# yeyupiaoling/MASR

Hardware: AMD Instinct MI355X
Metric: audio-seconds/sec (RTF^-1), conformer_streaming_fbank b32x10s, PCM->fbank->encoder->ctc_greedy->text (higher is better)
Workload: dtype f32; 1 GPU; configs[1]: conformer.yml streaming fbank, batch=32 synthetic 16 kHz 10 s utterances per GPU, ctc_greedy, random-init weights V=4233; global_batch=32, parallelism=dp1, world_size_observed=1, backend=none

## Files before the change

include/masr_hip.h:

```cpp
#ifndef MASR_HIP_H
#define MASR_HIP_H
#include <stdint.h>
#ifdef __cplusplus
extern "C" {
#endif

typedef struct masr_engine masr_engine;

typedef struct masr_config {
    int32_t model_kind;
    int32_t d_model;
    int32_t heads;
    int32_t d_ff;
    int32_t num_blocks;
    int32_t cnn_kernel;
    int32_t n_mels;
    int32_t vocab_size;
    int32_t causal;
    int32_t max_pos;
    int32_t device_id;
    int32_t reserved[5];
} masr_config;

const char* masr_last_error(void);
// ... 174 lines not shown
int masr_resample_plan(const masr_resample_feed* feeds, int32_t n_feeds, const masr_resample_rate* rates, int32_t n_rates,
                       int64_t src_bytes, int32_t dst_rows, int64_t dst_stride, int32_t* tiles, int64_t tiles_cap, int64_t* n_tiles,
                       int32_t* bad_feed, const char** why);
int masr_resample_feeds(masr_engine* e, const void* src_dev, int64_t src_bytes, const masr_resample_feed* feeds_host,
                        const masr_resample_feed* feeds_dev, int32_t n_feeds, const masr_resample_rate* rates_host,
                        const masr_resample_rate* rates_dev, int32_t n_rates, const int32_t* tiles_host, const int32_t* tiles_dev,
                        int64_t n_tiles, float* dst_dev, int32_t dst_rows, int64_t dst_stride, void* stream);
int masr_encode_chunk(masr_engine* e, const int32_t* stream_ids, int32_t n, const float* feats_dev, int32_t Tc,
                      float* probs_dev, int32_t* argmax_dev, float* maxprob_dev, void* stream);
int masr_stream_export_cache(masr_engine* e, int32_t stream_id, float* att_dev, float* cnn_dev, void* stream);

int masr_op_layernorm(masr_engine* e, const float* x_dev, const float* w_dev, const float* b_dev, float* y_dev,
                      int32_t M, float eps, void* stream);
int masr_op_gemm(masr_engine* e, const float* a_dev, const float* w_dev, const float* bias_dev, const float* res_dev,
                 float* c_dev, int32_t M, int32_t N, int32_t K, int32_t act, float alpha, void* stream);
int masr_op_ctc_collapse_rows(masr_engine* e, const int32_t* argmax_dev, const float* maxprob_dev, const int32_t* n_frames_dev,
                              const int32_t* in_rows_dev_or_null, int32_t ld_in, int32_t B, int32_t Tp, int32_t blank,
                              int32_t* rows_dev, void* stream);
int masr_op_beam_nbest(masr_engine* e, const int32_t* n_live_host, const int32_t* node_host, const int32_t* ch_host,
                       const float* score_host, const int32_t* pool_parent_host, const int32_t* pool_ch_host, int32_t B,
                       int32_t beam_size, int32_t pool_cap, int32_t nbest, int32_t* tokens_host, int32_t max_len, int32_t* len_host,
                       float* score_host_out, int32_t* count_host);
int masr_op_attention(masr_engine* e, const float* q_dev, const float* k_dev, const float* v_dev, float* out_dev,
                      const float* ptab_dev, int32_t n_pos, const float* bias_u_dev, const float* bias_v_dev, int32_t nseq,
                      const int64_t* q_off, const int64_t* k_off, const int64_t* v_off, const int64_t* out_off, const int32_t* nq,
                      const int32_t* nk, const int32_t* klen, const int32_t* pos0, const int32_t* q_abs0, int32_t heads,
                      int32_t q_stride, int32_t kv_stride, int32_t chunk_size, int32_t pos_stride, int32_t group, int32_t t_true,
                      void* stream);
int masr_op_attention_plain(masr_engine* e, const float* q_dev, const float* k_dev, const float* v_dev, float* out_dev, int32_t nseq,
                            const int64_t* q_off, const int64_t* k_off, const int64_t* v_off, const int64_t* out_off,
// ... 48 lines not shown
```

masr_amd/_lib.py:

```python
import collections
import contextlib
import ctypes as C
import os

import numpy as _np

from .build import LIB_PATH

_lib = None


class MasrConfig(C.Structure):
    _fields_ = [('model_kind', C.c_int32), ('d_model', C.c_int32), ('heads', C.c_int32), ('d_ff', C.c_int32),
                ('num_blocks', C.c_int32), ('cnn_kernel', C.c_int32), ('n_mels', C.c_int32),
                ('vocab_size', C.c_int32), ('causal', C.c_int32), ('max_pos', C.c_int32), ('device_id', C.c_int32),
                ('reserved', C.c_int32 * 5)]


class MasrError(RuntimeError):
    pass


_P = C.c_void_p
_I = C.c_int32
# ... 72 lines not shown
    'masr_resample_f32': [_P, C.c_int64, C.c_double, _P, _P, C.c_int64, _I, _P, C.c_int64],
    'masr_resample_rows': [_P, _P, _I, C.c_int64, _P, _P, _I, C.c_double, _P, C.c_int64, _I, _P, _I, C.c_int64, _P],
    'masr_resample_rate_fill': [C.c_double, _P, C.c_int64, _I, _P],
    'masr_resample_tile_span': [_P],
    'masr_resample_plan': [_P, _I, _P, _I, C.c_int64, _I, C.c_int64, _P, C.c_int64, C.POINTER(C.c_int64), C.POINTER(_I),
                           C.POINTER(C.c_char_p)],
    'masr_resample_feeds': [_P, _P, C.c_int64, _P, _P, _I, _P, _P, _I, _P, _P, C.c_int64, _P, _I, C.c_int64, _P],
    'masr_pool_set_rate': [_P, _I, C.c_double, _P, C.c_int64, _I, C.POINTER(_I)],
    'masr_pool_step_rates': [_P, _I, _P, _P, _P, _P, _P, _P, _P, _P, C.POINTER(_I), C.POINTER(_P), C.POINTER(_P), C.POINTER(_P),
                             C.POINTER(_I), C.POINTER(_P), _P],
    'masr_stream_set_history': [_P, _I, _I],
    'masr_encode_chunk': [_P, C.POINTER(_I), _I, _P, _I, _P, _P, _P, _P],
    'masr_stream_export_cache': [_P, _I, _P, _P, _P],
    'masr_op_layernorm': [_P, _P, _P, _P, _P, _I, _F, _P],
    'masr_op_gemm': [_P, _P, _P, _P, _P, _P, _I, _I, _I, _I, _F, _P],
    'masr_op_ctc_collapse_rows': [_P, _P, _P, _P, _P, _I, _I, _I, _I, _P, _P],
    'masr_op_attention': [_P, _P, _P, _P, _P, _P, _I, _P, _P, _I, _P, _P, _P, _P, _P, _P, _P, _P, _P, _I, _I, _I, _I, _I, _I, _I, _P],
    'masr_op_attention_plain': [_P, _P, _P, _P, _P, _I, _P, _P, _P, _P, _P, _P, _P, _P, _I, _I, _I, _I, _I, _P],
    'masr_decoder_enable': [_P, _I, _I, _I, _I],
    'masr_rescore': [_P, _P, _P, _I, _I, _P, _P, _I, _I, _I, _P, _P, _P],
    'masr_op_decoder_scores': [_P, _P, _P, _I, _I, _P, _P, _I, _I, _I, _P, _P, _P],
    'masr_decoder_info': [_P, C.POINTER(_I), C.POINTER(_I), C.POINTER(_I), C.POINTER(C.c_int64), C.POINTER(C.c_int64)],
    'masr_attention_decode': [_P, _P, _P, _I, _I, _I, _I, _P, _I, _P, _P, C.POINTER(_I), _P],
    'masr_op_decoder_step': [_P, _P, _P, _I, _I, _P, _P, _I, _I, _I, _P, _P, _P, _P],
    'masr_beam_search_batch_nbest': [_P, _P, _P, _P, _I, _I, _I, _I, _I, _I, _I, _P, _I, _P, _P, _P],
    'masr_beam_nbest_gpu': [_P, _I, _I, _I, _P, _F, _F, _P, _I, _P, _P, _P, _P],
    'masr_gbeam_nbest': [_P, _I, _I, _P, _I, _P, _P, _P, _P],
    'masr_op_beam_nbest': [_P, _P, _P, _P, _P, _P, _P, _I, _I, _I, _I, _P, _I, _P, _P, _P],
    'masr_side_stream': [_P, _I, C.POINTER(_P)],
    'masr_select_lane': [_P, _I],
# ... 30 lines not shown
                        f'(hipcc --offload-arch=gfx950). There is no CPU fallback.')
    h = C.CDLL(LIB_PATH)
    for name, args in SIGNATURES.items():
        fn = getattr(h, name)
        fn.argtypes = args
        fn.restype = _RESTYPE.get(name, C.c_int)
    _lib = h
    return h


def check(rc):
    if rc != 0:
        raise MasrError(lib().masr_last_error().decode('utf-8', 'replace'))


_ENGINE_KEYS = {'beam_profile': 2, 'prof_stride': 16, 'skip_padding': 38}


def debug_key_table():
    rows = []
    key, default, experimental, name = _I(), _I(), _I(), C.c_char_p()
    while lib().masr_debug_key_info(len(rows), C.byref(key), C.byref(default), C.byref(experimental), C.byref(name)) == 0:
        rows.append((key.value, name.value.decode(), default.value, bool(experimental.value)))
    return rows


FFN_KERNELS = ('X3', 'COOP', 'DUAL', 'ROWS16', 'PC')
FfnPlan = collections.namedtuple('FfnPlan', 'kernel nsplit cpb ny packed tail_in_kernel head_in_kernel split_head prof')


def ffn_plan(d_ff, M, keys=None, d_model=256, affine=0, tail_n=0, tail_planar=0, head_ktaps=0, head_norm=0):
# ... 19 lines not shown
```

masr_amd/build.py:

```python
import os
import subprocess
from concurrent.futures import ThreadPoolExecutor

ROOT = os.path.dirname(os.path.abspath(__file__))
CSRC = os.path.join(ROOT, 'csrc')
LIB_DIR = os.path.join(ROOT, 'lib')
LIB_PATH = os.path.join(LIB_DIR, 'libmasr_hip.so')
SOURCES = ['gemm_f32.hip', 'ffn_reduce.hip', 'ffn_pc.hip', 'sqz_layer.hip', 'rowgemm.hip', 'rowgemm_small.hip', 'elementwise.hip', 'wide.hip',
           'attention.hip', 'lstm.hip', 'gru.hip', 'beam_gpu.hip', 'beam_nbest.hip', 'lm_scorer.cpp', 'fbank.hip', 'silero.hip', 'engine.hip', 'pool.hip',
           'beam_search.cpp', 'stage.cpp', 'resample.cpp', 'resample.hip', 'knobs.cpp', 'decoder.hip', 'decoder_step.hip',
           'engine_attdecoder.hip', 'ctc_align.hip', 'engine_layers.hip', 'engine_conformer.hip', 'engine_efficient.hip',
           'engine_squeezeformer.hip', 'engine_ds2.hip', 'engine_ctc.hip', 'engine_frontend.hip', 'engine_ops.hip']
EXPERIMENTS = os.environ.get('MASR_BUILD_EXPERIMENTS') == '1'
EXPERIMENT_SOURCES = ['gemm_bf16x3.hip', 'ffn_x3.hip', 'ffn_coop.hip', 'ffn_dual.hip']
if EXPERIMENTS:
    SOURCES = SOURCES + EXPERIMENT_SOURCES
HEADERS = [os.path.join(CSRC, 'common.h'), os.path.join(CSRC, 'knobs.h'), os.path.join(CSRC, 'ffn_plan.h'),
           os.path.join(CSRC, 'lm_scorer.h'), os.path.join(CSRC, 'engine_state.h'), os.path.join(CSRC, 'engine_encoder.h'),
           os.path.join(os.path.dirname(ROOT), 'include', 'masr_hip.h')]
FLAGS = ['--offload-arch=gfx950', '-O3', '-std=c++17', '-fPIC', '-Wno-unused-value'] + (['-DMASR_EXPERIMENTS=1'] if EXPERIMENTS else [])
FILE_FLAGS = {'resample.hip': ['-ffp-contract=off', '-fno-gpu-flush-denormals-to-zero']}
STAMP = os.path.join(LIB_DIR, '.build_flavour')


# ... 84 lines not shown
```

masr_amd/csrc/common.h:

```cpp
#pragma once
#include <hip/hip_runtime.h>
#include <stdint.h>

#include "knobs.h"
#include "lm_scorer.h"

struct masr_resample_feed;
struct masr_resample_rate;

#ifndef MASR_EXPERIMENTS
#define MASR_EXPERIMENTS 0
#endif

typedef float f32x4 __attribute__((ext_vector_type(4)));
typedef float f32x16 __attribute__((ext_vector_type(16)));

namespace masr {

struct LdsAttr {
    size_t granted[32] = {};
};
void ensure_dynamic_lds(const void* fn, size_t bytes, LdsAttr& st);
void note_launch_error(const char* what, hipError_t e);

// ... 151 lines not shown
void launch_export_cnn_layer(const float* cache, float* out, int used, int total, int d, hipStream_t s);
void launch_export_att_planar(const float* kplane, const float* vplane, float* out, int H, int t, int dk, hipStream_t s);
void launch_affine_rows(const float* x, const float* w, const float* b, float* y, int M, int seq_t, int pad, hipStream_t s);
void launch_export_cnn(const float* cache, float* out, int L, int pad, int d, hipStream_t s);

struct AttSeq;
enum RowGemmPro { RG_PRO_PLAIN = 0, RG_PRO_LN = 1, RG_PRO_LN_PAD = 2, RG_PRO_AFFINE = 3,
                  RG_PRO_HIST = 4, RG_PRO_DWCONV = 5 };
enum RowGemmEpi { RG_EPI_STORE = 0, RG_EPI_RESID = 1, RG_EPI_GLU = 2, RG_EPI_CTC = 3, RG_EPI_CHAIN = 4 };
struct RowGemmArgs {
    const float* A;
    const float* lnw;
    const float* lnb;
    const float* W;
    const float* Wp;
    const float* bias;
    float* C;
    const float* R;
    float* R2;
    const int* lens;
    int* out_idx;
    float* out_maxp;
    int M, N;
    int lda, ldc, ldr;
    float eps, alpha;
    int seq_t, pad;
    int mask_tp;
    int mstride;
    int out_seq_t;
    int out_pad_l, out_pad_tot;
    int plane_cols;
    long plane_stride;
    int a_seq_t, a_seq_stride;
    float* const* cache_rd;
    float* const* cache_wr;
    int hist_affine;
    const float* dw_w;
    const float* dw_b;
    const float* gconst;
    const AttSeq* kv_seqs;
    int kv_tq;
};
bool launch_rowgemm(const RowGemmArgs& a, int pro, int epi, hipStream_t s);
bool launch_rowgemm_small(const RowGemmArgs& a, int pro, int epi, hipStream_t s);

struct FfnPostLn {
    const float* lnw;
    const float* lnb;
    float* y;
    float eps = 1e-5f;
};
struct FfnTail {
    const float* lnw;
    const float* lnb;
    const float* W;
    const float* bias;
    float* out;
    int N, ldo;
    const float* pre_lnw;
// ... 274 lines not shown
```

masr_amd/csrc/engine_conformer.hip:

```cpp
#include "engine_encoder.h"

namespace masr {

int finalize_conformer(masr_engine* e, hipStream_t s) {
    const int d = e->cfg.d_model, dff = e->cfg.d_ff, L = e->cfg.num_blocks, V = e->cfg.vocab_size, F = e->cfg.n_mels;
    const int il = e->input_layer, H = e->cfg.heads, dk = d / H;
    CHK(upload_conv_frontend(e, "encoder.embed.conv.0", "encoder.embed.conv.2", il == IL_CONV2D6 ? 5 : 3,
                             il == IL_CONV2D8 ? "encoder.embed.conv.4" : nullptr));
    if (il != IL_CONV2D && e->host.count("encoder.embed.out.0.weight"))
        return fail("input_layer conv2d6 / conv2d8 but the checkpoint holds encoder.embed.out.0 (a conv2d front-end)");
    if (il == IL_CONV2D && e->host.count("encoder.embed.linear.weight"))
        return fail("input_layer conv2d but the checkpoint holds encoder.embed.linear (a conv2d6 / conv2d8 front-end)");
    if (il != IL_CONV2D8 && e->host.count("encoder.embed.conv.4.weight"))
        return fail("the checkpoint holds a third subsampling conv (encoder.embed.conv.4, conv2d8) but input_layer is not conv2d8");
    CHK(upload_embed_proj(e, il == IL_CONV2D ? "encoder.embed.out.0" : "encoder.embed.linear", sub_bins(il, F)));
    CHK(upload_pos_table(e));
    e->layers.assign(L, LayerW{});
    for (int i = 0; i < L; ++i) {
        LayerW& w = e->layers[i];
        const std::string p = "encoder.encoders." + std::to_string(i) + ".";
        CHK(up_wb(e, p + "norm_ff_macaron", {d}, &w.ln_ffm_w, &w.ln_ffm_b));
        CHK(up_wb(e, p + "norm_mha", {d}, &w.ln_mha_w, &w.ln_mha_b));
        CHK(up_wb(e, p + "norm_conv", {d}, &w.ln_conv_w, &w.ln_conv_b));
        CHK(up_wb(e, p + "norm_ff", {d}, &w.ln_ff_w, &w.ln_ff_b));
// ... 169 lines not shown
            launch_attention(e->attseq.as<AttSeq>(), B, Tq, H, 3 * d, 3 * d, w.ptab, w.pos_u, w.pos_v, chunk, 1, s, 256, att_pos(e));
        }
        if (few_rows) {
            mhsa_out(e, s, w, M);
            const bool fuse = knobs().split_head && e->cfg.cnn_kernel == 15 && knobs().ffn_packed >= 2 && !knobs().no_ffn_head;
            CHK(conv_module(e, s, w, ctx, false, 0, 4, false, fuse));
            FfnArgs f2 = ffn_final(w, M, x);
            if (fuse) f2.head = conv_head(e, w, feat_lens_dev, Tq, e->cfg.cnn_kernel, 4);
            CHK(ffn(e, s, f2));
            continue;
        } else if (knobs().no_chain) {
            mhsa_out(e, s, w, M);
            CHK(conv_module(e, s, w, ctx, false));
            CHK(ffn(e, s, ffn_final(w, M)));
        } else {
            if (!fuse_ac) mhsa_out_pw1(e, s, w, ctx);
            FfnArgs f2 = ffn_final(w, M);
            f2.head = conv_head(e, w, feat_lens_dev, Tq, e->cfg.cnn_kernel, 4);
            CHK(ffn(e, s, f2));
        }
        prev = &w;
    }
    if (prev) launch_layernorm(x, prev->ln_fin_w, prev->ln_fin_b, x, M, 1e-5f, 0, 0, nullptr, s);
    launch_layernorm(x, e->after_w, e->after_b, enc_out_dev, M, 1e-5f, 0, 0, nullptr, s);
    LAUNCHCHK();
    return 0;
}

int encode_chunk_conformer(masr_engine* e, hipStream_t s, std::vector<Stream*>& st, const float* feats_dev, int Tc,
                                  float* probs_dev, int32_t* argmax_dev, float* maxprob_dev) {
    const int n = (int)st.size();
// ... 65 lines not shown
```

masr_amd/csrc/engine_encoder.h:

```cpp
#pragma once
#include "engine_state.h"

#pragma GCC visibility push(hidden)
namespace masr {

struct EncodeCtx {
    int nseq;
    int Tq;
    const int* lens;
};

struct FfnDone {
    int err;
    bool tail_done = false;
    bool head_done = false;
    FfnDone(int err_ = 0) : err(err_) {}
    operator int() const { return err; }
};

struct ChunkWindow {
    int cache_t1, first_full;
    int next_cache_t1, ncs;
};

// ... 37 lines not shown
FfnArgs ffn_of(int M, const float* lnw, const float* lnb, const float* w1, const float* b1, const float* w2, const float* b2);
FfnTail qkv_tail(const masr_engine* e, const LayerW& w, float* out, int ldo);
FfnHead conv_head(const masr_engine* e, const LayerW& w, const int* lens, int Tq, int ktaps, int mstride);
FfnDone ffn(masr_engine* e, hipStream_t s, FfnArgs a);
int embed(masr_engine* e, hipStream_t s, const float* feats, int nseq, int T, int* Tq_out, const int* skip_lens = nullptr);
int ensure_layer_ws(masr_engine* e, int nseq, int Tq);
int conv_module(masr_engine* e, hipStream_t s, const LayerW& w, const EncodeCtx& c, bool hist, int K = 0, int mstride = 4,
                bool pw1_done = false, bool pw2_later = false);
int conv_module_stream(masr_engine* e, hipStream_t s, const LayerW& w, int n, int Tq, float* const* cache_rd,
                       float* const* cache_wr, int K, bool pw2_later = false);
void qkv_proj(masr_engine* e, hipStream_t s, int pro, const float* lnw, const float* lnb, const float* wqkv, const float* bqkv, int M,
              const AttSeq* kv_seqs = nullptr, int kv_tq = 0);
void mhsa(masr_engine* e, hipStream_t s, const LayerW& w, int M, const AttSeq* kv_seqs = nullptr, int kv_tq = 0);
void mhsa_out(masr_engine* e, hipStream_t s, const LayerW& w, int M);
void mhsa_out_pw1(masr_engine* e, hipStream_t s, const LayerW& w, const EncodeCtx& c, int mstride = 4, int K = 0,
                  const float* att = nullptr, int a_seq_t = 0, int a_seq_stride = 0);
int upload_conv_frontend(masr_engine* e, const std::string& c1, const std::string& c2, int ks, const char* c3, int d = 0);
int upload_embed_proj(masr_engine* e, const std::string& proj, int F2);
int upload_pos_table(masr_engine* e);
int get_conv_bn(masr_engine* e, const std::string& p, const HostTensor* bn[4]);
int upload_qkv(masr_engine* e, const std::string& p, float** wqkv, float** bqkv);
int upload_depthwise(masr_engine* e, const std::string& p, int K, float** dw_w, float** dw_b);
int build_ptab(masr_engine* e, hipStream_t s, const float* wpos, float** ptab);
int upload_gconst(masr_engine* e, hipStream_t s, const float* pw1_b, bool wide, float** gconst);
ChunkWindow chunk_window(const Stream& st, int T0);
int half_rate_window(const Stream& st, int want, int* first, int* count);
AttSeq interleaved_seq(const float* q, float* cache, int d, int first, int ncached, int Tl, float* out, int pos0, int q_abs0);
std::vector<float*> cnn_cache_table(const std::vector<Stream*>& st, int L, size_t layer_floats);
int upload_chunk_tables(masr_engine* e, hipStream_t s, const std::vector<AttSeq>& hs, const std::vector<float*>& hp,
                        void* third_dev = nullptr, const void* third = nullptr, size_t third_bytes = 0);
void advance_half_rate(std::vector<Stream*>& st, const std::vector<ChunkWindow>& win, int T0, int Tr);
// ... 18 lines not shown
```

masr_amd/csrc/engine_layers.hip:

```cpp
#include "engine_encoder.h"

namespace masr {

void gemm(masr_engine* e, hipStream_t s, const float* A, int lda, const float* W, const float* bias, float* C, int ldc,
          int M, int N, int K, int act, float alpha, const float* R, int ldr, int kind,
          const int* lens, int mask_tp) {
    GemmArgs a{};
    a.A = A; a.W = W; a.bias = bias; a.C = C; a.R = R; a.lens = lens;
    a.M = M; a.N = N; a.K = K; a.lda = lda; a.ldc = ldc; a.ldr = ldr;
    a.act = act; a.alpha = alpha; a.mask_tp = mask_tp;
    ProfScope ps(e, s, kind, 2.0 * M * (double)N * K);
    if (knobs().bf16x3 && launch_gemm_bf16x3(a, A_PLAIN, s)) return;
    launch_gemm(a, A_PLAIN, EPI_STD, s);
}

int enc_dim(const masr_engine* e) {
    return e->cfg.model_kind == 3 ? e->cfg.d_model * (e->cfg.causal ? 1 : 2) : e->cfg.d_model;
}
int layer_kernel(const masr_engine* e, int i) {
    return (e->cfg.model_kind == 2 && e->stride_idx >= 0 && i > e->stride_idx) ? e->cfg.cnn_kernel / 2 : e->cfg.cnn_kernel;
}
bool layer_grouped(const masr_engine* e, int i) { return e->cfg.model_kind == 2 && i < e->n_group_layers; }

RowGemmArgs rg_args(const float* A, int lda, const float* W, const float* bias, float* C, int ldc, int M, int N) {
// ... 316 lines not shown
void qkv_proj(masr_engine* e, hipStream_t s, int pro, const float* lnw, const float* lnb, const float* wqkv, const float* bqkv, int M,
              const AttSeq* kv_seqs, int kv_tq) {
    const int d = e->cfg.d_model;
    RowGemmArgs g = rg_args(e->x.as<float>(), d, wqkv, bqkv, e->qkv.as<float>(), 3 * d, M, 3 * d);
    g.lnw = lnw; g.lnb = lnb; g.kv_seqs = kv_seqs; g.kv_tq = kv_tq;
    rowgemm(e, s, pro, RG_EPI_STORE, g);
}
void mhsa(masr_engine* e, hipStream_t s, const LayerW& w, int M, const AttSeq* kv_seqs, int kv_tq) {
    qkv_proj(e, s, RG_PRO_LN, w.ln_mha_w, w.ln_mha_b, w.wqkv, w.bqkv, M, kv_seqs, kv_tq);
}
void mhsa_out(masr_engine* e, hipStream_t s, const LayerW& w, int M) {
    resid_gemm(e, s, e->att.as<float>(), w.wo, w.bo, e->x.as<float>(), M);
}

void mhsa_out_pw1(masr_engine* e, hipStream_t s, const LayerW& w, const EncodeCtx& c, int mstride, int K,
                  const float* att, int a_seq_t, int a_seq_stride) {
    const int d = e->cfg.d_model, pad = (K > 0 ? K : e->cfg.cnn_kernel) - 1, M = c.nseq * c.Tq;
    float* x = e->x.as<float>();
    RowGemmArgs a{};
    a.A = att ? att : e->att.as<float>(); a.lda = d; a.a_seq_t = a_seq_t; a.a_seq_stride = a_seq_stride; a.lnw = w.ln_conv_w; a.lnb = w.ln_conv_b; a.W = w.chain_w; a.bias = w.chain_b;
    a.C = e->glu.as<float>(); a.ldc = d; a.M = M; a.N = 3 * d; a.R = x; a.R2 = x; a.ldr = d; a.alpha = 1.f;
    a.lens = c.lens; a.seq_t = c.Tq; a.mstride = mstride; a.eps = 1e-5f;
    a.out_seq_t = c.Tq; a.out_pad_l = e->cfg.causal ? pad : pad / 2; a.out_pad_tot = pad;
    if (knobs().rowgemm_packed) a.Wp = packed_rows_of(e, w.chain_w, 3 * d, s);
    ProfScope ps(e, s, PROF_GEMM, 2.0 * M * (double)(3 * d) * d);
    launch_rowgemm(a, RG_PRO_PLAIN, RG_EPI_CHAIN, s);
}

static int upload_conv_kxk(masr_engine* e, const std::string& name, int d, int ks, float** wd, float** bd) {
    const int kk = ks * ks;
    const HostTensor* t;
    CHK(get(e, name + ".weight", {d, d, ks, ks}, &t));
    std::vector<float> w((size_t)d * kk * d);
    for (int co = 0; co < d; ++co)
        for (int ci = 0; ci < d; ++ci)
            for (int k = 0; k < kk; ++k)
                w[(size_t)co * kk * d + (size_t)(ci / 32) * kk * 32 + k * 32 + ci % 32] = t->v[((size_t)co * d + ci) * kk + k];
    CHK(upload(e, w, wd));
    return up(e, name + ".bias", {d}, bd);
// ... 168 lines not shown
```

masr_amd/csrc/engine_ops.hip:

```cpp
#include "engine_encoder.h"

using namespace masr;

extern "C" {

int masr_op_layernorm(masr_engine* e, const float* x_dev, const float* w_dev, const float* b_dev, float* y_dev,
                      int32_t M, float eps, void* stream) {
    if (!e) return fail("null engine");
    ENTER(e);
    launch_layernorm(x_dev, w_dev, b_dev, y_dev, M, eps, 0, 0, nullptr, (hipStream_t)stream);
    LAUNCHCHK();
    return 0;
}

int masr_op_gemm(masr_engine* e, const float* a_dev, const float* w_dev, const float* bias_dev, const float* res_dev,
                 float* c_dev, int32_t M, int32_t N, int32_t K, int32_t act, float alpha, void* stream) {
    if (!gemm_act_valid(act))
        return fail("masr_op_gemm: act = " + std::to_string(act) + " is not an activation: 0 = none, 1 = relu, 2 = silu, 3 = gelu, "
                    "4 = tanh, 5 = hardtanh, 6 = selu");
    if (!e) return fail("null engine");
    ENTER(e);
    CallGuard call_guard(e, (hipStream_t)stream);
    if (K % 32) return fail("K must be a multiple of 32");
    gemm(e, (hipStream_t)stream, a_dev, K, w_dev, bias_dev, c_dev, N, M, N, K, act, alpha, res_dev, N);
    LAUNCHCHK();
    return 0;
}

}

static int op_attention(masr_engine* e, int pos_mode, const float* q_dev, const float* k_dev, const float* v_dev, float* out_dev,
                      const float* ptab_dev, int32_t n_pos, const float* bias_u_dev, const float* bias_v_dev, int32_t nseq,
                      const int64_t* q_off, const int64_t* k_off, const int64_t* v_off, const int64_t* out_off, const int32_t* nq,
                      const int32_t* nk, const int32_t* klen, const int32_t* pos0, const int32_t* q_abs0, int32_t heads,
                      int32_t q_stride, int32_t kv_stride, int32_t chunk_size, int32_t pos_stride, int32_t group, int32_t t_true,
                      void* stream) {
    const bool pos = pos_mode == ATT_REL_POS;
    if (!q_dev || !k_dev || !v_dev || !out_dev || (pos && (!ptab_dev || !bias_u_dev || !bias_v_dev)) || !q_off || !k_off || !v_off ||
        !out_off || !nq || !nk || !klen || !pos0 || !q_abs0)
// ... 75 lines not shown
                            int32_t q_stride, int32_t kv_stride, int32_t chunk_size, int32_t pos_stride, void* stream) {
    if (nseq <= 0) return fail("masr_op_attention: nseq must be positive");
    const std::vector<int32_t> pos0((size_t)nseq, 0);
    return op_attention(e, ATT_NO_POS, q_dev, k_dev, v_dev, out_dev, nullptr, 0, nullptr, nullptr, nseq, q_off, k_off, v_off, out_off, nq,
                        nk, klen, pos0.data(), q_abs0, heads, q_stride, kv_stride, chunk_size, pos_stride, 1, 0, stream);
}

int masr_debug_set(masr_engine* e, int32_t key, int32_t value) {
    if (!e) return fail("null engine");
    const KnobInfo* k = knob_find(key);
    if (k) {
        if (!MASR_EXPERIMENTS && k->experimental && value != 0)
            return fail("masr_debug_set: this key selects an experimental kernel that is not in this build (MASR_BUILD_EXPERIMENTS=1)");
        knob_set(key, value);
    } else if (key == 38) e->skip_padding = value;
    else if (key == 16) { e->prof_stride = value > 1 ? value : 1; e->prof_seen = 0; }
    else if (key == 2) {
        if (value) {
            if (!e->beam_prof) {
                void* p = nullptr;
                HIPCHK(hipMalloc(&p, 16 * sizeof(long long)));
                e->owned.push_back(p);
                e->beam_prof = (long long*)p;
            }
        } else if (e->beam_prof) {
            long long h[16];
            HIPCHK(hipMemcpy(h, e->beam_prof, sizeof(h), hipMemcpyDeviceToHost));
            fprintf(stderr, "beam phases (cycles, last workgroup): setup+hash %lld  extensions %lld  prefixes+count %lld  select %lld  compact %lld\n",
                    h[0], h[1], h[2], h[3], h[4]);
            fprintf(stderr, "  narrow step (%lld frames): tables+candidates %lld  hash+contexts %lld  children+scorer table %lld  extensions %lld  "
                    "prefixes+select %lld  scan %lld  survivors %lld  new prefixes %lld\n", h[5], h[6], h[7], h[8], h[9], h[10], h[11], h[12], h[13]);
            if (h[15] > 0) fprintf(stderr, "  wide step (%lld frames): %.1f distinct scorer contexts per frame\n", h[15], (double)h[14] / (double)h[15]);
            e->beam_prof = nullptr;
        }
    }
    else return fail("unknown debug key");
    return 0;
}

int masr_debug_reset(masr_engine* e) {
    if (!e) return fail("null engine");
    knobs_reset();
    e->skip_padding = 7;
    e->prof_stride = 1;
    e->prof_seen = 0;
    return 0;
}

int masr_debug_key_info(int32_t index, int32_t* key, int32_t* default_value, int32_t* experimental, const char** name) {
    const KnobInfo* k = knob_info(index);
    if (!k) return 1;
    if (key) *key = k->key;
    if (default_value) *default_value = knob_default(*k);
    if (experimental) *experimental = k->experimental;
    if (name) *name = k->name;
    return 0;
}

// ... 42 lines not shown
```

masr_amd/csrc/engine_state.h:

```cpp
#pragma once
#include <math.h>
#include <stdio.h>
#include <string.h>

#include <algorithm>
#include <map>
#include <string>
#include <utility>
#include <vector>

#include "../../include/masr_hip.h"
#include "common.h"
#include "ffn_plan.h"

namespace masr {
int engine_fail(const std::string& m);
int subsampled_frames(const masr_engine* e, int feature_frames);
}

#pragma GCC visibility push(hidden)
namespace masr {
inline int fail(const std::string& m) { return engine_fail(m); }
bool launch_error_pending();
std::string take_launch_error();
// ... 224 lines not shown
    bool pack_pending = false;
    bool finalized = false;
    std::map<std::string, masr::HostTensor> host;
    std::vector<void*> owned;
    float *cmvn_mean = nullptr, *cmvn_istd = nullptr, *conv1_w = nullptr, *conv1_b = nullptr, *conv2_w = nullptr,
          *conv2_b = nullptr, *conv3_w = nullptr, *conv3_b = nullptr, *embed_w = nullptr, *embed_b = nullptr, *after_w = nullptr, *after_b = nullptr,
          *ctc_w = nullptr, *ctc_b = nullptr, *pe = nullptr;
    std::vector<masr::LayerW> layers;
    std::vector<masr::SqLayerW> sq_layers;
    std::vector<masr::Ds2LayerW> ds2_layers;
    std::vector<masr::GBeam> gbeams;
    masr::DevBuf beam_pool, beam_state;
    std::map<void*, std::pair<masr::DevBuf, masr::DevBuf>> beam_ws;
    std::map<void*, masr::BeamLast> beam_last;
    std::map<void*, masr::DevBuf> ms_ws;
    int skip_padding = 7;
    void* beam_first_stream = nullptr;
    bool beam_first_set = false;
    std::map<std::pair<int, const float*>, masr::PackedW> packed;
    long long* beam_prof = nullptr;
    float *preln_w = nullptr, *preln_b = nullptr, *tr_dw_w = nullptr, *tr_dw_b = nullptr, *tr_pw_w = nullptr,
          *tr_pw_b = nullptr, *rec_w = nullptr, *rec_b = nullptr;
    int reduce_idx = -1, recover_idx = -1;
    int stride_idx = -1, n_group_layers = 0, group_size = 3;
    int input_layer = masr::IL_CONV2D;
    bool conv_bn = false;
    bool ds2_gru = false;
    int pos_enc = masr::POS_ENC_REL;
    int act = masr::ENC_ACT_SWISH;
    float *window = nullptr, *melwt = nullptr, *tw512 = nullptr, *twr4 = nullptr;
// ... 85 lines not shown
```

masr_amd/csrc/rowgemm.hip:

```cpp
#include <cstdio>
#include <cstdlib>

#include "common.h"

namespace masr {

static constexpr int RG_BM = 32;
static constexpr int RG_K = 256;
static constexpr int RG_ALD = RG_K + 4;
static constexpr int RG_WLD = 32 + 4;
static constexpr int RG_WSLAB = 32 * RG_WLD;
static constexpr int RG_NSET = 4;

__device__ __forceinline__ float rg_wsum(float v) {
    return wave_sum_dpp(v);
}

template <int PRO, int EPI, int GSPLIT, int PACKED = 0>
__global__ __launch_bounds__(512) void rowgemm_kernel(RowGemmArgs p) {
    extern __shared__ __align__(16) float sm[];
    float* at = sm;
    float* wpv = at + RG_BM * RG_ALD;
    float* red = wpv + 8 * 2 * RG_WSLAB;

    const int tid = threadIdx.x, lane = tid & 63;
    const int wave = __builtin_amdgcn_readfirstlane(tid >> 6);
    const int frow = lane & 31, fh = lane >> 5;
    const int row0 = blockIdx.x * RG_BM;
    float* wmine = wpv + wave * 2 * RG_WSLAB;

    {
        f32x4 gw = f32x4{1.f, 1.f, 1.f, 1.f}, gb = f32x4{0.f, 0.f, 0.f, 0.f};
        if (PRO != RG_PRO_PLAIN) {
            gw = *reinterpret_cast<const f32x4*>(p.lnw + lane * 4);
            gb = *reinterpret_cast<const f32x4*>(p.lnb + lane * 4);
        }
        f32x4 v4[4];
        bool live4[4];
// ... 320 lines not shown
            }
            float S = 0.f;
#pragma unroll
            for (int w = 0; w < 8; ++w) {
                const float* d = red + (w * RG_BM + tid) * 3;
                S += d[1] * __expf(d[0] - M);
            }
            p.out_idx[row0 + tid] = I;
            p.out_maxp[row0 + tid] = 1.0f / S;
        }
    }
}

template <int PRO, int EPI>
static void launch_rg(const RowGemmArgs& a, hipStream_t s) {
    const size_t lds = (size_t)(RG_BM * RG_ALD + 8 * 2 * RG_WSLAB + (EPI == RG_EPI_CHAIN ? RG_BM * RG_ALD : 8 * RG_BM * 3)) * sizeof(float);
    constexpr bool can_split = EPI == RG_EPI_STORE || EPI == RG_EPI_RESID;
    static LdsAttr attr0, attr1;
    ensure_dynamic_lds(reinterpret_cast<const void*>(rowgemm_kernel<PRO, EPI, 0>), lds, attr0);
    if (can_split) ensure_dynamic_lds(reinterpret_cast<const void*>(rowgemm_kernel<PRO, EPI, can_split ? 1 : 0>), lds, attr1);
    const int rowblocks = (a.M + RG_BM - 1) / RG_BM, ngroups = (a.N + 255) / 256;
    if (EPI != RG_EPI_CTC && a.N % 256 != 0) {
        fprintf(stderr, "rowgemm: N must be a multiple of 256 for this epilogue\n");
        abort();
    }
    constexpr bool can_pack = true;
    if (can_split && ngroups > 1 && rowblocks < 64) {
        hipLaunchKernelGGL((rowgemm_kernel<PRO, EPI, can_split ? 1 : 0>), dim3(rowblocks, ngroups), dim3(512), lds, s, a);
    } else if (can_pack && a.Wp) {
        static LdsAttr attrp;
        ensure_dynamic_lds(reinterpret_cast<const void*>(rowgemm_kernel<PRO, EPI, 0, can_pack ? 1 : 0>), lds, attrp);
        hipLaunchKernelGGL((rowgemm_kernel<PRO, EPI, 0, can_pack ? 1 : 0>), dim3(rowblocks), dim3(512), lds, s, a);
    } else {
        hipLaunchKernelGGL((rowgemm_kernel<PRO, EPI, 0>), dim3(rowblocks), dim3(512), lds, s, a);
    }
}

static void launch_rowgemm_big(const RowGemmArgs& a, int pro, int epi, hipStream_t s) {
    if (pro == RG_PRO_LN && epi == RG_EPI_STORE) launch_rg<RG_PRO_LN, RG_EPI_STORE>(a, s);
    else if (pro == RG_PRO_PLAIN && epi == RG_EPI_STORE) launch_rg<RG_PRO_PLAIN, RG_EPI_STORE>(a, s);
    else if (pro == RG_PRO_PLAIN && epi == RG_EPI_RESID) launch_rg<RG_PRO_PLAIN, RG_EPI_RESID>(a, s);
    else if (pro == RG_PRO_LN_PAD && epi == RG_EPI_GLU) launch_rg<RG_PRO_LN_PAD, RG_EPI_GLU>(a, s);
    else if (pro == RG_PRO_PLAIN && epi == RG_EPI_GLU) launch_rg<RG_PRO_PLAIN, RG_EPI_GLU>(a, s);
    else if (pro == RG_PRO_AFFINE && epi == RG_EPI_STORE) launch_rg<RG_PRO_AFFINE, RG_EPI_STORE>(a, s);
    else if (pro == RG_PRO_AFFINE && epi == RG_EPI_GLU) launch_rg<RG_PRO_AFFINE, RG_EPI_GLU>(a, s);
    else if (pro == RG_PRO_PLAIN && epi == RG_EPI_CTC) launch_rg<RG_PRO_PLAIN, RG_EPI_CTC>(a, s);
    else if (pro == RG_PRO_LN && epi == RG_EPI_CTC) launch_rg<RG_PRO_LN, RG_EPI_CTC>(a, s);
    else if (pro == RG_PRO_PLAIN && epi == RG_EPI_CHAIN) launch_rg<RG_PRO_PLAIN, RG_EPI_CHAIN>(a, s);
}

bool launch_rowgemm(const RowGemmArgs& a, int pro, int epi, hipStream_t s) {
    if (a.M <= 0 || a.N <= 0) return true;
    if (knobs().rowgemm_small && launch_rowgemm_small(a, pro, epi, s)) return true;
    if (pro == RG_PRO_HIST || pro == RG_PRO_DWCONV) return false;
    launch_rowgemm_big(a, pro, epi, s);
    if (a.kv_seqs && epi == RG_EPI_STORE) launch_kv_append(a.kv_seqs, a.C, a.M / a.kv_tq, a.kv_tq, s);
    return true;
}

}
```

Before: 52780 audio-seconds/sec.

## Add 16-row MFMA chain kernel for MHSA-out, LN and pointwise GLU fusion

Adds a dedicated chain16 kernel that uses 16-row tiles and f32 MFMA 16x16x4 with a register-ring prefetch of a 16-row packed weight layout. It fuses the attention output projection plus residual, the conv LayerNorm, and the pointwise conv GLU for d_model 256. It is enabled by default for the streaming conformer path. It also shrinks dynamic LDS for the existing packed rowgemm variant by dropping the unused weight slab, which can raise occupancy. Smaller row tiles give more blocks for small M, but each block reuses the weights across fewer rows.

```diff
diff --git a/include/masr_hip.h b/include/masr_hip.h
--- a/include/masr_hip.h
+++ b/include/masr_hip.h
@@ -212,6 +212,8 @@
                       int32_t M, float eps, void* stream);
 int masr_op_gemm(masr_engine* e, const float* a_dev, const float* w_dev, const float* bias_dev, const float* res_dev,
                  float* c_dev, int32_t M, int32_t N, int32_t K, int32_t act, float alpha, void* stream);
+int masr_op_chain(masr_engine* e, int32_t layer, const float* att_dev, float* x_dev, float* glu_dev, const int32_t* lens_dev_or_null,
+                  int32_t nseq, int32_t Tq, void* stream);
 int masr_op_ctc_collapse_rows(masr_engine* e, const int32_t* argmax_dev, const float* maxprob_dev, const int32_t* n_frames_dev,
                               const int32_t* in_rows_dev_or_null, int32_t ld_in, int32_t B, int32_t Tp, int32_t blank,
                               int32_t* rows_dev, void* stream);
diff --git a/masr_amd/_lib.py b/masr_amd/_lib.py
--- a/masr_amd/_lib.py
+++ b/masr_amd/_lib.py
@@ -110,6 +110,7 @@
     'masr_stream_export_cache': [_P, _I, _P, _P, _P],
     'masr_op_layernorm': [_P, _P, _P, _P, _P, _I, _F, _P],
     'masr_op_gemm': [_P, _P, _P, _P, _P, _P, _I, _I, _I, _I, _F, _P],
+    'masr_op_chain': [_P, _I, _P, _P, _P, _P, _I, _I, _P],
     'masr_op_ctc_collapse_rows': [_P, _P, _P, _P, _P, _I, _I, _I, _I, _P, _P],
     'masr_op_attention': [_P, _P, _P, _P, _P, _P, _I, _P, _P, _I, _P, _P, _P, _P, _P, _P, _P, _P, _P, _I, _I, _I, _I, _I, _I, _I, _P],
     'masr_op_attention_plain': [_P, _P, _P, _P, _P, _I, _P, _P, _P, _P, _P, _P, _P, _P, _I, _I, _I, _I, _I, _P],
@@ -170,7 +171,7 @@
         raise MasrError(lib().masr_last_error().decode('utf-8', 'replace'))
 
 
-_ENGINE_KEYS = {'beam_profile': 2, 'prof_stride': 16, 'skip_padding': 38}
+_ENGINE_KEYS = {'beam_profile': 2, 'prof_stride': 16, 'skip_padding': 38, 'chain16': 45}
 
 
 def debug_key_table():
diff --git a/masr_amd/build.py b/masr_amd/build.py
--- a/masr_amd/build.py
+++ b/masr_amd/build.py
@@ -6,7 +6,7 @@
 CSRC = os.path.join(ROOT, 'csrc')
 LIB_DIR = os.path.join(ROOT, 'lib')
 LIB_PATH = os.path.join(LIB_DIR, 'libmasr_hip.so')
-SOURCES = ['gemm_f32.hip', 'ffn_reduce.hip', 'ffn_pc.hip', 'sqz_layer.hip', 'rowgemm.hip', 'rowgemm_small.hip', 'elementwise.hip', 'wide.hip',
+SOURCES = ['gemm_f32.hip', 'ffn_reduce.hip', 'ffn_pc.hip', 'sqz_layer.hip', 'rowgemm.hip', 'rowgemm16.hip', 'rowgemm_small.hip', 'elementwise.hip', 'wide.hip',
            'attention.hip', 'lstm.hip', 'gru.hip', 'beam_gpu.hip', 'beam_nbest.hip', 'lm_scorer.cpp', 'fbank.hip', 'silero.hip', 'engine.hip', 'pool.hip',
            'beam_search.cpp', 'stage.cpp', 'resample.cpp', 'resample.hip', 'knobs.cpp', 'decoder.hip', 'decoder_step.hip',
            'engine_attdecoder.hip', 'ctc_align.hip', 'engine_layers.hip', 'engine_conformer.hip', 'engine_efficient.hip',
diff --git a/masr_amd/csrc/common.h b/masr_amd/csrc/common.h
--- a/masr_amd/csrc/common.h
+++ b/masr_amd/csrc/common.h
@@ -189,6 +189,7 @@
     const float* lnb;
     const float* W;
     const float* Wp;
+    const float* Wp16;
     const float* bias;
     float* C;
     const float* R;
@@ -218,6 +219,7 @@
 };
 bool launch_rowgemm(const RowGemmArgs& a, int pro, int epi, hipStream_t s);
 bool launch_rowgemm_small(const RowGemmArgs& a, int pro, int epi, hipStream_t s);
+void launch_chain16(const RowGemmArgs& a, hipStream_t s);
 
 struct FfnPostLn {
     const float* lnw;
diff --git a/masr_amd/csrc/engine_conformer.hip b/masr_amd/csrc/engine_conformer.hip
--- a/masr_amd/csrc/engine_conformer.hip
+++ b/masr_amd/csrc/engine_conformer.hip
@@ -207,7 +207,7 @@
             CHK(conv_module(e, s, w, ctx, false));
             CHK(ffn(e, s, ffn_final(w, M)));
         } else {
-            if (!fuse_ac) mhsa_out_pw1(e, s, w, ctx);
+            if (!fuse_ac) mhsa_out_pw1(e, s, w, ctx, 4, 0, nullptr, 0, 0, true);
             FfnArgs f2 = ffn_final(w, M);
             f2.head = conv_head(e, w, feat_lens_dev, Tq, e->cfg.cnn_kernel, 4);
             CHK(ffn(e, s, f2));
diff --git a/masr_amd/csrc/engine_encoder.h b/masr_amd/csrc/engine_encoder.h
--- a/masr_amd/csrc/engine_encoder.h
+++ b/masr_amd/csrc/engine_encoder.h
@@ -75,7 +75,8 @@
 void mhsa(masr_engine* e, hipStream_t s, const LayerW& w, int M, const AttSeq* kv_seqs = nullptr, int kv_tq = 0);
 void mhsa_out(masr_engine* e, hipStream_t s, const LayerW& w, int M);
 void mhsa_out_pw1(masr_engine* e, hipStream_t s, const LayerW& w, const EncodeCtx& c, int mstride = 4, int K = 0,
-                  const float* att = nullptr, int a_seq_t = 0, int a_seq_stride = 0);
+                  const float* att = nullptr, int a_seq_t = 0, int a_seq_stride = 0, bool rows16 = false,
+                  float* x_io = nullptr, float* glu_out = nullptr);
 int upload_conv_frontend(masr_engine* e, const std::string& c1, const std::string& c2, int ks, const char* c3, int d = 0);
 int upload_embed_proj(masr_engine* e, const std::string& proj, int F2);
 int upload_pos_table(masr_engine* e);
diff --git a/masr_amd/csrc/engine_layers.hip b/masr_amd/csrc/engine_layers.hip
--- a/masr_amd/csrc/engine_layers.hip
+++ b/masr_amd/csrc/engine_layers.hip
@@ -354,15 +354,18 @@
 }
 
 void mhsa_out_pw1(masr_engine* e, hipStream_t s, const LayerW& w, const EncodeCtx& c, int mstride, int K,
-                  const float* att, int a_seq_t, int a_seq_stride) {
+                  const float* att, int a_seq_t, int a_seq_stride, bool rows16, float* x_io, float* glu_out) {
     const int d = e->cfg.d_model, pad = (K > 0 ? K : e->cfg.cnn_kernel) - 1, M = c.nseq * c.Tq;
-    float* x = e->x.as<float>();
+    float* x = x_io ? x_io : e->x.as<float>();
     RowGemmArgs a{};
     a.A = att ? att : e->att.as<float>(); a.lda = d; a.a_seq_t = a_seq_t; a.a_seq_stride = a_seq_stride; a.lnw = w.ln_conv_w; a.lnb = w.ln_conv_b; a.W = w.chain_w; a.bias = w.chain_b;
-    a.C = e->glu.as<float>(); a.ldc = d; a.M = M; a.N = 3 * d; a.R = x; a.R2 = x; a.ldr = d; a.alpha = 1.f;
+    a.C = glu_out ? glu_out : e->glu.as<float>(); a.ldc = d; a.M = M; a.N = 3 * d; a.R = x; a.R2 = x; a.ldr = d; a.alpha = 1.f;
     a.lens = c.lens; a.seq_t = c.Tq; a.mstride = mstride; a.eps = 1e-5f;
     a.out_seq_t = c.Tq; a.out_pad_l = e->cfg.causal ? pad : pad / 2; a.out_pad_tot = pad;
-    if (knobs().rowgemm_packed) a.Wp = packed_rows_of(e, w.chain_w, 3 * d, s);
+    if (knobs().rowgemm_packed) {
+        if (rows16 && e->chain16 && a_seq_t == 0) a.Wp16 = packed_rows_of(e, w.chain_w, 3 * d, s, PACK_ROWS16);
+        else a.Wp = packed_rows_of(e, w.chain_w, 3 * d, s);
+    }
     ProfScope ps(e, s, PROF_GEMM, 2.0 * M * (double)(3 * d) * d);
     launch_rowgemm(a, RG_PRO_PLAIN, RG_EPI_CHAIN, s);
 }
diff --git a/masr_amd/csrc/engine_ops.hip b/masr_amd/csrc/engine_ops.hip
--- a/masr_amd/csrc/engine_ops.hip
+++ b/masr_amd/csrc/engine_ops.hip
@@ -23,6 +23,21 @@
     CallGuard call_guard(e, (hipStream_t)stream);
     if (K % 32) return fail("K must be a multiple of 32");
     gemm(e, (hipStream_t)stream, a_dev, K, w_dev, bias_dev, c_dev, N, M, N, K, act, alpha, res_dev, N);
+    LAUNCHCHK();
+    return 0;
+}
+
+int masr_op_chain(masr_engine* e, int32_t layer, const float* att_dev, float* x_dev, float* glu_dev, const int32_t* lens_dev_or_null,
+                  int32_t nseq, int32_t Tq, void* stream) {
+    if (!att_dev || !x_dev || !glu_dev) return fail("masr_op_chain: null argument");
+    if (nseq <= 0 || Tq <= 0) return fail("masr_op_chain: nseq and Tq must be positive");
+    if (!e) return fail("null engine");
+    ENTER(e);
+    if (e->cfg.model_kind != 0 || e->cfg.d_model != 256 || layer < 0 || layer >= (int)e->layers.size() || !e->layers[layer].chain_w)
+        return fail("masr_op_chain: a Conformer engine of output_size 256 and one of its layers");
+    CallGuard call_guard(e, (hipStream_t)stream);
+    mhsa_out_pw1(e, (hipStream_t)stream, e->layers[layer], EncodeCtx{nseq, Tq, lens_dev_or_null}, 4, 0, att_dev, 0, 0, true, x_dev,
+                 glu_dev);
     LAUNCHCHK();
     return 0;
 }
@@ -128,6 +143,7 @@
             return fail("masr_debug_set: this key selects an experimental kernel that is not in this build (MASR_BUILD_EXPERIMENTS=1)");
         knob_set(key, value);
     } else if (key == 38) e->skip_padding = value;
+    else if (key == 45) e->chain16 = value;
     else if (key == 16) { e->prof_stride = value > 1 ? value : 1; e->prof_seen = 0; }
     else if (key == 2) {
         if (value) {
@@ -156,6 +172,7 @@
     if (!e) return fail("null engine");
     knobs_reset();
     e->skip_padding = 7;
+    e->chain16 = 1;
     e->prof_stride = 1;
     e->prof_seen = 0;
     return 0;
diff --git a/masr_amd/csrc/engine_state.h b/masr_amd/csrc/engine_state.h
--- a/masr_amd/csrc/engine_state.h
+++ b/masr_amd/csrc/engine_state.h
@@ -262,6 +262,7 @@
     std::map<void*, std::pair<masr::DevBuf, masr::DevBuf>> beam_ws;
     std::map<void*, masr::BeamLast> beam_last;
     std::map<void*, masr::DevBuf> ms_ws;
+    int chain16 = 1;
     int skip_padding = 7;
     void* beam_first_stream = nullptr;
     bool beam_first_set = false;
diff --git a/masr_amd/csrc/rowgemm.hip b/masr_amd/csrc/rowgemm.hip
--- a/masr_amd/csrc/rowgemm.hip
+++ b/masr_amd/csrc/rowgemm.hip
@@ -11,6 +11,10 @@
 static constexpr int RG_WLD = 32 + 4;
 static constexpr int RG_WSLAB = 32 * RG_WLD;
 static constexpr int RG_NSET = 4;
+__host__ __device__ constexpr int rg_slab_floats(int packed) { return packed ? 0 : 8 * 2 * RG_WSLAB; }
+__host__ __device__ constexpr int rg_lds_floats(int epi, int packed) {
+    return RG_BM * RG_ALD + rg_slab_floats(packed) + (epi == RG_EPI_CHAIN ? RG_BM * RG_ALD : 8 * RG_BM * 3);
+}
 
 __device__ __forceinline__ float rg_wsum(float v) {
     return wave_sum_dpp(v);
@@ -21,7 +25,7 @@
     extern __shared__ __align__(16) float sm[];
     float* at = sm;
     float* wpv = at + RG_BM * RG_ALD;
-    float* red = wpv + 8 * 2 * RG_WSLAB;
+    float* red = wpv + rg_slab_floats(PACKED);
 
     const int tid = threadIdx.x, lane = tid & 63;
     const int wave = __builtin_amdgcn_readfirstlane(tid >> 6);
@@ -372,7 +376,7 @@
 
 template <int PRO, int EPI>
 static void launch_rg(const RowGemmArgs& a, hipStream_t s) {
-    const size_t lds = (size_t)(RG_BM * RG_ALD + 8 * 2 * RG_WSLAB + (EPI == RG_EPI_CHAIN ? RG_BM * RG_ALD : 8 * RG_BM * 3)) * sizeof(float);
+    const size_t lds = (size_t)rg_lds_floats(EPI, 0) * sizeof(float), lds_packed = (size_t)rg_lds_floats(EPI, 1) * sizeof(float);
     constexpr bool can_split = EPI == RG_EPI_STORE || EPI == RG_EPI_RESID;
     static LdsAttr attr0, attr1;
     ensure_dynamic_lds(reinterpret_cast<const void*>(rowgemm_kernel<PRO, EPI, 0>), lds, attr0);
@@ -387,8 +391,8 @@
         hipLaunchKernelGGL((rowgemm_kernel<PRO, EPI, can_split ? 1 : 0>), dim3(rowblocks, ngroups), dim3(512), lds, s, a);
     } else if (can_pack && a.Wp) {
         static LdsAttr attrp;
-        ensure_dynamic_lds(reinterpret_cast<const void*>(rowgemm_kernel<PRO, EPI, 0, can_pack ? 1 : 0>), lds, attrp);
-        hipLaunchKernelGGL((rowgemm_kernel<PRO, EPI, 0, can_pack ? 1 : 0>), dim3(rowblocks), dim3(512), lds, s, a);
+        ensure_dynamic_lds(reinterpret_cast<const void*>(rowgemm_kernel<PRO, EPI, 0, can_pack ? 1 : 0>), lds_packed, attrp);
+        hipLaunchKernelGGL((rowgemm_kernel<PRO, EPI, 0, can_pack ? 1 : 0>), dim3(rowblocks), dim3(512), lds_packed, s, a);
     } else {
         hipLaunchKernelGGL((rowgemm_kernel<PRO, EPI, 0>), dim3(rowblocks), dim3(512), lds, s, a);
     }
@@ -404,7 +408,10 @@
     else if (pro == RG_PRO_AFFINE && epi == RG_EPI_GLU) launch_rg<RG_PRO_AFFINE, RG_EPI_GLU>(a, s);
     else if (pro == RG_PRO_PLAIN && epi == RG_EPI_CTC) launch_rg<RG_PRO_PLAIN, RG_EPI_CTC>(a, s);
     else if (pro == RG_PRO_LN && epi == RG_EPI_CTC) launch_rg<RG_PRO_LN, RG_EPI_CTC>(a, s);
-    else if (pro == RG_PRO_PLAIN && epi == RG_EPI_CHAIN) launch_rg<RG_PRO_PLAIN, RG_EPI_CHAIN>(a, s);
+    else if (pro == RG_PRO_PLAIN && epi == RG_EPI_CHAIN) {
+        if (a.Wp16 && a.a_seq_t == 0 && a.N == 768) launch_chain16(a, s);
+        else launch_rg<RG_PRO_PLAIN, RG_EPI_CHAIN>(a, s);
+    }
 }
 
 bool launch_rowgemm(const RowGemmArgs& a, int pro, int epi, hipStream_t s) {
diff --git a/masr_amd/csrc/rowgemm16.hip b/masr_amd/csrc/rowgemm16.hip
--- /dev/null
+++ b/masr_amd/csrc/rowgemm16.hip
@@ -0,0 +1,152 @@
+#include "common.h"
+
+namespace masr {
+
+static constexpr int C16_BM = 16;
+static constexpr int C16_K = 256;
+static constexpr int C16_ALD = C16_K + 4;
+static constexpr int C16_RING = 8;
+static constexpr int C16_NFRAG = 3 * 32;
+__host__ __device__ constexpr int c16_k0(int kk) { return (kk & 1) * 4 + (kk >> 1); }
+
+__global__ __launch_bounds__(512) __attribute__((amdgpu_waves_per_eu(4))) void chain16_kernel(RowGemmArgs p) {
+    extern __shared__ __align__(16) float sm[];
+    float* at = sm;
+    float* red = at + C16_BM * C16_ALD;
+
+    const int tid = threadIdx.x, lane = tid & 63;
+    const int wave = __builtin_amdgcn_readfirstlane(tid >> 6);
+    const int fr = lane & 15, kk = lane >> 4, ko = c16_k0(kk);
+    const int row0 = blockIdx.x * C16_BM;
+    const int lr_last = p.M - 1 - row0;
+
+    {
+        f32x4 v4[2];
+#pragma unroll
+        for (int rr = 0; rr < 2; ++rr) {
+            const int row = row0 + min(wave * 2 + rr, lr_last);
+            v4[rr] = *reinterpret_cast<const f32x4*>(p.A + (size_t)row * p.lda + lane * 4);
+        }
+#pragma unroll
+        for (int rr = 0; rr < 2; ++rr) {
+            const int lr = wave * 2 + rr;
+            *reinterpret_cast<f32x4*>(&at[lr * C16_ALD + lane * 4]) = lr <= lr_last ? v4[rr] : f32x4{0.f, 0.f, 0.f, 0.f};
+        }
+    }
+
+    const unsigned lane16 = lane * 16;
+    const __amdgpu_buffer_rsrc_t prs =
+        __builtin_amdgcn_make_buffer_rsrc(const_cast<float*>(p.Wp16), 0, 3 * 256 * C16_K * 4, 0x00020000);
+    auto pld = [&](int t, int f) -> f32x4 {
+        const unsigned fi = (unsigned)((t * 8 + wave) * 32 + f) * 256u;
+        return __builtin_bit_cast(f32x4, __builtin_amdgcn_raw_buffer_load_b128(prs, lane16, fi * 4u, 0));
+    };
+    f32x4 pre[C16_RING];
+#pragma unroll
+    for (int k = 0; k < C16_RING; ++k) pre[k] = pld(0, k);
+
+    const int cb0 = p.seq_t > 0 ? row0 / p.seq_t : 0, ct0 = p.seq_t > 0 ? row0 - cb0 * p.seq_t : 0;
+    const int ob0 = p.out_seq_t > 0 ? row0 / p.out_seq_t : 0, ot0 = p.out_seq_t > 0 ? row0 - ob0 * p.out_seq_t : 0;
+    float res0[8], cbo[2], cba[2], cbg[2];
+#pragma unroll
+    for (int nt = 0; nt < 2; ++nt) {
+        const int ch = wave * 32 + 16 * nt + fr;
+        cbo[nt] = p.bias[ch];
+        cba[nt] = p.bias[256 + ch];
+        cbg[nt] = p.bias[512 + ch];
+#pragma unroll
+        for (int r = 0; r < 4; ++r) res0[4 * nt + r] = p.R[(size_t)(row0 + min(4 * kk + r, lr_last)) * p.ldr + ch];
+    }
+    const f32x4 cgw = *reinterpret_cast<const f32x4*>(p.lnw + lane * 4);
+    const f32x4 cgb = *reinterpret_cast<const f32x4*>(p.lnb + lane * 4);
+    __syncthreads();
+
+    const float* xa = at + fr * C16_ALD + ko;
+    f32x4 accv[2];
+#pragma unroll
+    for (int t = 0; t < 3; ++t) {
+        f32x4 acc[2] = {{0.f, 0.f, 0.f, 0.f}, {0.f, 0.f, 0.f, 0.f}};
+        float a0 = xa[0], a1 = xa[2];
+#pragma unroll
+        for (int g = 0; g < 32; ++g) {
+            float n0 = 0.f, n1 = 0.f;
+            if (g + 1 < 32) { n0 = xa[8 * (g + 1)]; n1 = xa[8 * (g + 1) + 2]; }
+#pragma unroll
+            for (int q = 0; q < 4; ++q) {
+                acc[q & 1] = __builtin_amdgcn_mfma_f32_16x16x4f32(q < 2 ? a0 : a1, pre[g % C16_RING][q], acc[q & 1], 0, 0, 0);
+                if (q == 3 && t * 32 + g + C16_RING < C16_NFRAG) pre[g % C16_RING] = pld(t + (g + C16_RING) / 32, (g + C16_RING) & 31);
+                __builtin_amdgcn_sched_barrier(0);
+            }
+            a0 = n0;
+            a1 = n1;
+        }
+
+        if (t == 0) {
+#pragma unroll
+            for (int nt = 0; nt < 2; ++nt) {
+                const int ch = wave * 32 + 16 * nt + fr;
+                const float bv = cbo[nt];
+#pragma unroll
+                for (int r = 0; r < 4; ++r) {
+                    const int lr = 4 * kk + r;
+                    const float v = res0[4 * nt + r] + (acc[nt][r] + bv);
+                    if (lr <= lr_last) p.R2[(size_t)(row0 + lr) * p.ldr + ch] = v;
+                    red[lr * C16_ALD + ch] = v;
+                }
+            }
+            __syncthreads();
+            {
+                const f32x4 gw = cgw, gb = cgb;
+#pragma unroll
+                for (int rr = 0; rr < 2; ++rr) {
+                    const int lr = wave * 2 + rr;
+                    bool live = lr <= lr_last;
+                    if (live && p.lens && p.seq_t > 0) {
+                        const SeqRow q = seq_row(cb0, ct0, p.seq_t, lr);
+                        live = p.mstride * q.t < p.lens[q.b];
+                    }
+                    const f32x4 v = *reinterpret_cast<const f32x4*>(&red[lr * C16_ALD + lane * 4]);
+                    const float mean = wave_sum_dpp(v[0] + v[1] + v[2] + v[3]) * (1.0f / 256.0f);
+                    const float d0 = v[0] - mean, d1 = v[1] - mean, d2 = v[2] - mean, d3 = v[3] - mean;
+                    const float var = wave_sum_dpp(d0 * d0 + d1 * d1 + d2 * d2 + d3 * d3) * (1.0f / 256.0f);
+                    const float rstd = 1.0f / sqrtf(var + p.eps);
+                    f32x4 o;
+                    o[0] = d0 * rstd * gw[0] + gb[0];
+                    o[1] = d1 * rstd * gw[1] + gb[1];
+                    o[2] = d2 * rstd * gw[2] + gb[2];
+                    o[3] = d3 * rstd * gw[3] + gb[3];
+                    if (!live) o = f32x4{0.f, 0.f, 0.f, 0.f};
+                    *reinterpret_cast<f32x4*>(&red[lr * C16_ALD + lane * 4]) = o;
+                }
+            }
+            __syncthreads();
+            xa = red + fr * C16_ALD + ko;
+        } else if (t == 1) {
+            accv[0] = acc[0];
+            accv[1] = acc[1];
+        } else {
+#pragma unroll
+            for (int r = 0; r < 4; ++r) {
+                const int lr = 4 * kk + r;
+                if (lr > lr_last) continue;
+                size_t crow = row0 + lr;
+                if (p.out_seq_t > 0) {
+                    const SeqRow q = seq_row(ob0, ot0, p.out_seq_t, lr);
+                    crow = (size_t)q.b * (p.out_seq_t + p.out_pad_tot) + p.out_pad_l + q.t;
+                }
+#pragma unroll
+                for (int nt = 0; nt < 2; ++nt) {
+                    const float g = acc[nt][r] + cbg[nt];
+                    p.C[crow * p.ldc + wave * 32 + 16 * nt + fr] = (accv[nt][r] + cba[nt]) * __builtin_amdgcn_rcpf(1.0f + __expf(-g));
+                }
+            }
+        }
+    }
+}
+
+void launch_chain16(const RowGemmArgs& a, hipStream_t s) {
+    const size_t lds = (size_t)2 * C16_BM * C16_ALD * sizeof(float);
+    hipLaunchKernelGGL(chain16_kernel, dim3((a.M + C16_BM - 1) / C16_BM), dim3(512), lds, s, a);
+}
+
+}
```

New measurement: 53070 audio-seconds/sec (median of 6 runs). About the same (+0.5%).
